# tarepan/DDSP-SVC-official

Measured on AMD Instinct MI355X. Metric: audio samples/sec @44.1kHz CombSub synth, higher is better.
Workload: dtype f32 storage and accumulation; products of the GEMM / FIR contractions split-bf16x3 (hi*hi+hi*lo+lo*hi), of the attention split-bf16 from three pieces (6 products) for the feature projections and two (3 products) for the context sums; everything else f32; `value_fp32_mfma` is the leg with every produ; 1 GPU; CombSub 44.1 kHz, batch=64x2 s per GPU (Fr=172, T=88064), units/f0/volume/spk_id -> audio, seeded random weights, in-kernel noise

## Files before the change

ddsp-svc-official_amd/csrc/fir_synth.hip:

```cpp
#include "gemm_f32.h"
#include "tables.h"

#include <stdlib.h>

namespace {

__global__ void __launch_bounds__(256) fir_act_kernel(int mode, const float* __restrict__ ctrl, int64_t ld, int M,
                                                      int ldo, int64_t rows, float* __restrict__ out, int split) {
    const int lane = threadIdx.x & 63;
    const int64_t row = (int64_t)blockIdx.x * 4 + (threadIdx.x >> 6);
    if (row >= rows) return;
    const float* src = ctrl + row * ld;
    if (mode != DDSP_FIR_ALLPASS) {
        float* dst = out + row * ldo;
        const float scale = (mode == DDSP_FIR_STATIC) ? (1.0f / 128.0f) : 1.0f;
        if (split) {
            for (int f0 = 0; f0 < M; f0 += 64) {
                const int f = f0 + lane;
                const float v = f < M ? expf(src[f]) * scale : 0.f;
                const uint32_t w = ddsp_split1_group8(v, lane);
                if (f < M) ((uint32_t*)dst)[f] = w;
            }
            return;
        }
        for (int f = lane; f < M; f += 64) dst[f] = expf(src[f]) * scale;
        return;
    }
    float* dst = out + row * ldo;
    const float pi_f = 3.14159274101257324f;
    double carry = 0.0;
    for (int f0 = 0; f0 < M; f0 += 64) {
        const int f = f0 + lane;
        const float gd = (f < M) ? __fmul_rn(pi_f, tanhf(src[f])) : 0.f;
        double incl = (double)gd;
#pragma unroll
        for (int o = 1; o < 64; o <<= 1) {
            double nb = __shfl_up(incl, o, 64);
            if (lane >= o) incl += nb;
        }
        const float phi = (float)(carry + incl);
        carry += __shfl(incl, 63, 64);
        float s = 0.f, c = 0.f;
        if (f < M) sincosf(phi, &s, &c);
        if (split) {
            const uint32_t wc = ddsp_split1_group8(c, lane), ws = ddsp_split1_group8(s, lane);
            if (f < M) {
                ((uint32_t*)dst)[f] = wc;
                ((uint32_t*)dst)[M + f] = ws;
            }
        } else if (f < M) {
            dst[f] = c;
            dst[M + f] = s;
        }
    }
}

struct EpiDynWindow {
    float* ir;
    int n;
    const float* f0;
    float sr15;
    int fast;
    __device__ __forceinline__ float col(int) const { return 0.f; }
    __device__ __forceinline__ float window_fast(float inv_hw, int k) const {
        float w = (float)(k - n / 2) * inv_hw;
        if (w > 1.0f) w = 0.0f;
        return fmaf(0.5f, __builtin_amdgcn_cosf(0.5f * w), 0.5f);
    }
    __device__ __forceinline__ float window(float hw, int k) const {
        float w = __fdiv_rn((float)(k - n / 2), hw);
        if (w > 1.0f) w = 0.0f;
        return __fdiv_rn(__fadd_rn(1.0f, cosf(__fmul_rn(3.14159274101257324f, w))), 2.0f);
    }
    __device__ __forceinline__ void operator()(int, int m, int k, float v, float) const {
        float* row = ir + (int64_t)m * n;
        if (fast) {
            const float inv_hw = __fdiv_rn(__fadd_rn(f0[m], 1e-3f), sr15);
            row[k] = v * window_fast(inv_hw, k);
            if (k > 0 && k < n / 2) row[n - k] = v * window_fast(inv_hw, n - k);
            return;
        }
        const float hw = __fdiv_rn(sr15, __fadd_rn(f0[m], 1e-3f));
        row[k] = __fmul_rn(v, window(hw, k));
        if (k > 0 && k < n / 2) row[n - k] = __fmul_rn(v, window(hw, n - k));
    }
};

struct EpiMirrorStore {
    float* ir;
    int n;
    __device__ __forceinline__ float col(int) const { return 0.f; }
    __device__ __forceinline__ void operator()(int, int m, int k, float v, float) const {
        float* row = ir + (int64_t)m * n;
        row[k] = v;
        if (k > 0 && k < n / 2) row[n - k] = v;
    }
};


__global__ void __launch_bounds__(256) fir_act_exp8_kernel(float scale, const float* __restrict__ ctrl, int64_t ld, int M, int ldo,
                                                           int64_t rows, float* __restrict__ out, int split) {
    const int per_row = M / 8;
    const int64_t i = (int64_t)blockIdx.x * 256 + threadIdx.x;
    if (i >= rows * per_row) return;
    const int64_t row = i / per_row;
    const int gq = (int)(i % per_row);
    const float* src = ctrl + row * ld + 8 * gq;
    const f32x4 a = *(const f32x4*)src, b = *(const f32x4*)(src + 4);
    float v[8];
#pragma unroll
    for (int e = 0; e < 4; ++e) {
        v[e] = expf(a[e]) * scale;
        v[4 + e] = expf(b[e]) * scale;
    }
    float* dst = out + row * ldo + 8 * gq;
    if (split) {
        ddsp_u32x4 hi, lo;
        ddsp_split8(v, hi, lo);
        *(ddsp_u32x4*)dst = hi;
        *(ddsp_u32x4*)(dst + 4) = lo;
    } else {
        *(f32x4*)dst = f32x4{v[0], v[1], v[2], v[3]};
        *(f32x4*)(dst + 4) = f32x4{v[4], v[5], v[6], v[7]};
    }
}

template <int CTRL, int ROW_MASK>
__device__ __forceinline__ double act_dpp_d(double v) {
    const uint64_t u = __builtin_bit_cast(uint64_t, v);
    const int lo = __builtin_amdgcn_update_dpp(0, (int)(uint32_t)u, CTRL, ROW_MASK, 0xf, false);
    const int hi = __builtin_amdgcn_update_dpp(0, (int)(uint32_t)(u >> 32), CTRL, ROW_MASK, 0xf, false);
    return __builtin_bit_cast(double, ((uint64_t)(uint32_t)hi << 32) | (uint32_t)lo);
}
__global__ void __launch_bounds__(256) fir_act_allpass4_kernel(const float* __restrict__ ctrl, int64_t ld, int M, int ldo, int64_t rows,
                                                               float* __restrict__ out, int split) {
    const int lane = threadIdx.x & 63;
    const int64_t row = (int64_t)blockIdx.x * 4 + (threadIdx.x >> 6);
    if (row >= rows) return;
    const float* src = ctrl + row * ld;
    float* dst = out + row * ldo;
    const float pi_f = 3.14159274101257324f;
    double carry = 0.0;
    for (int f0 = 0; f0 < M; f0 += 256) {
        const int f = f0 + 4 * lane;
        const bool in = f < M;
        f32x4 x = {0.f, 0.f, 0.f, 0.f};
        if (in) x = *(const f32x4*)(src + f);
        double run = 0.0, loc[4];
#pragma unroll
        for (int e = 0; e < 4; ++e) {
            const float gd = in ? __fmul_rn(pi_f, tanhf(x[e])) : 0.f;
            run += (double)gd;
            loc[e] = run;
        }
        double incl = run;
        incl += act_dpp_d<0x111, 0xf>(incl);
        incl += act_dpp_d<0x112, 0xf>(incl);
        incl += act_dpp_d<0x114, 0xf>(incl);
        incl += act_dpp_d<0x118, 0xf>(incl);
        incl += act_dpp_d<0x142, 0xa>(incl);
        incl += act_dpp_d<0x143, 0xc>(incl);
        const double base = carry + (incl - run);
        f32x4 c, sn;
#pragma unroll
        for (int e = 0; e < 4; ++e) {
            const float phi = (float)(base + loc[e]);
            float s_ = 0.f, c_ = 0.f;
            if (in) sincosf(phi, &s_, &c_);
            c[e] = c_;
            sn[e] = s_;
        }
        {
            const uint64_t u = __builtin_bit_cast(uint64_t, incl);
            const uint32_t lo = __builtin_amdgcn_readlane((int)(uint32_t)u, 63), hi = __builtin_amdgcn_readlane((int)(uint32_t)(u >> 32), 63);
            carry += __builtin_bit_cast(double, ((uint64_t)hi << 32) | lo);
        }
        if (split) {
            const ddsp_u32x4 pc = ddsp_split4_pair(c, (lane & 1) != 0, 1), ps = ddsp_split4_pair(sn, (lane & 1) != 0, 1);
            if (in) {
                *(ddsp_u32x4*)(dst + f) = pc;
                *(ddsp_u32x4*)(dst + M + f) = ps;
            }
        } else if (in) {
            *(f32x4*)(dst + f) = c;
            *(f32x4*)(dst + M + f) = sn;
        }
    }
}

__global__ void __launch_bounds__(256) repack_rows_kernel(const float* __restrict__ src, int n, int64_t rows, int ld,
                                                          float* __restrict__ dst) {
    typedef float f32x2r __attribute__((ext_vector_type(2)));
    const int half = ld / 2;
    const int64_t total = rows * half;
    for (int64_t i = (int64_t)blockIdx.x * blockDim.x + threadIdx.x; i < total; i += (int64_t)gridDim.x * blockDim.x) {
        const int64_t m = i / half;
        const int k = 2 * (int)(i % half);
        f32x2r v = {0.f, 0.f};
        if (k < n) v = *(const f32x2r*)(src + m * n + k);
        *(f32x2r*)(dst + m * ld + k) = v;
    }
}

__global__ void __launch_bounds__(256) dyn_window_scale_kernel(float* __restrict__ d_ir, const float* __restrict__ f0,
                                                               int n, int64_t rows, float sr15) {
    const int64_t total = rows * n;
    for (int64_t i = (int64_t)blockIdx.x * blockDim.x + threadIdx.x; i < total; i += (int64_t)gridDim.x * blockDim.x) {
        const int64_t m = i / n;
        const int k = (int)(i % n);
        const float hw = __fdiv_rn(sr15, __fadd_rn(f0[m], 1e-3f));
        float w = __fdiv_rn((float)(k - n / 2), hw);
        if (w > 1.0f) w = 0.0f;
        d_ir[i] *= __fdiv_rn(__fadd_rn(1.0f, cosf(__fmul_rn(3.14159274101257324f, w))), 2.0f);
    }
}

__global__ void __launch_bounds__(256) fir_act_bwd_kernel(int mode, const float* __restrict__ ctrl, int64_t ld, int M,
                                                          const float* __restrict__ d_act, int lda, int64_t rows,
// ... 38 lines not shown
    }
    float tail = 0.f;
#pragma unroll
    for (int c = 15; c >= 0; --c) {
        if (c < nchunk) {
            float incl = dphi[c];
#pragma unroll
            for (int o = 1; o < 64; o <<= 1) {
                float nb = __shfl_down(incl, o, 64);
                if (lane + o < 64) incl += nb;
            }
            const float G = incl + tail;
            tail += __shfl(incl, 0, 64);
            const int f = c * 64 + lane;
            if (f < M) dst[f] = G * pi_f * (1.0f - th[c] * th[c]);
        }
    }
}

}


extern "C" int ddsp_fir_from_ctrl(ddsp_ctx* ctx, void* stream, int mode, const float* ctrl, int64_t ctrl_ld,
                                  int n_mag, const float* f0_frames, int64_t rows, int sr, float* ir) {
    DDSP_REQUIRE(ctx, ctx && ctrl && ir, "ddsp_fir_from_ctrl: null argument");
    DDSP_REQUIRE(ctx, mode >= 0 && mode <= 2, "ddsp_fir_from_ctrl: unknown mode");
    DDSP_REQUIRE(ctx, n_mag >= 3 && n_mag <= 1024 && ctrl_ld >= n_mag && rows >= 0 && rows < (1 << 30),
                 "ddsp_fir_from_ctrl: bad shape");
    DDSP_REQUIRE(ctx, mode != DDSP_FIR_DYNAMIC || f0_frames, "ddsp_fir_from_ctrl: DYNAMIC needs f0_frames");
    if (rows == 0) return DDSP_OK;
    hipStream_t st = (hipStream_t)stream;
    DDSP_ENTER_DEVICE(ctx);
    const int M = n_mag, n = 2 * (n_mag - 1);
    const int K = (mode == DDSP_FIR_ALLPASS) ? 2 * M : M;
    const int lda = ddsp_pad4(K);
    int rc = ddsp_scratch_reserve_bytes(ctx, (size_t)rows * lda * sizeof(float) + 4096);
    if (rc) return rc;
    ddsp_scratch_reset(ctx);
    float* act = nullptr;
    rc = ddsp_scratch_get(ctx, (size_t)rows * lda * sizeof(float), (void**)&act);
    if (rc) return rc;
    float* tab = nullptr;
    const int kind = mode == DDSP_FIR_ALLPASS ? TAB_IRDFT_CPLX : (mode == DDSP_FIR_STATIC ? TAB_IRDFT_RE_HANN : TAB_IRDFT_RE);
    const bool tap_major = K % 32 == 0;
    rc = ddsp_get_table(ctx, st, kind, M, tap_major ? 1 : 0, &tab);
    if (rc) return rc;
    float* tab_split = nullptr;
    if (tap_major && ctx->math != DDSP_MATH_FP32 && (rc = ddsp_get_table(ctx, st, kind, M, 2, &tab_split))) return rc;

    const bool presplit = tap_major && tab_split && rows >= 8192 && M % 8 == 0 && ctx->math != 4;
    ddsp_prof_begin(ctx, st, PF_FIR_ACT);
    const bool wide = M % 8 == 0 && ctrl_ld % 4 == 0 && lda % 8 == 0 && ((uintptr_t)ctrl % 16) == 0;
    if (wide && mode != DDSP_FIR_ALLPASS)
        hipLaunchKernelGGL(fir_act_exp8_kernel, dim3((unsigned)ceil_div64(rows * (M / 8), 256)), dim3(256), 0, st,
                           mode == DDSP_FIR_STATIC ? 1.0f / 128.0f : 1.0f, ctrl, ctrl_ld, M, lda, rows, act, presplit ? 1 : 0);
    else if (wide)
        hipLaunchKernelGGL(fir_act_allpass4_kernel, dim3((unsigned)ceil_div64(rows, 4)), dim3(256), 0, st, ctrl, ctrl_ld, M, lda, rows,
                           act, presplit ? 1 : 0);
    else
        hipLaunchKernelGGL(fir_act_kernel, dim3((unsigned)ceil_div64(rows, 4)), dim3(256), 0, st, mode, ctrl, ctrl_ld, M,
                           lda, rows, act, presplit ? 1 : 0);
    ddsp_prof_end(ctx, st, 0.0, 4.0 * rows * (M + K));
    DDSP_LAUNCH_CHECK(ctx);
    ddsp_prof_begin(ctx, st, PF_FIR_DFT_GEMM);

    auto run = [&](gemm::Args g, const auto& epi) {
        g.math = tap_major ? (ctx->math == 4 ? DDSP_MATH_SPLIT_BF16 : ctx->math) : 0;
        g.B_split = tab_split;
        if (presplit) {
            g.A_split = 1;
            g.B = tab_split;
        }
        if (tap_major)
            gemm::launch<true, true, gemm::A_PLAIN>(st, g, 1, epi);
        else
            gemm::launch<true, false, gemm::A_PLAIN>(st, g, 1, epi);
    };
    const int64_t ldb = tap_major ? K : ddsp_pad4(n);
    if (mode == DDSP_FIR_ALLPASS) {
        gemm::Args g = gemm::make(act, lda, tab, ldb, (int)rows, n, K);
        run(g, gemm::EpiStore{ir, n, nullptr, 1, 0, 0});
    } else {
        gemm::Args g = gemm::make(act, lda, tab, ldb, (int)rows, n / 2 + 1, K);
        if (mode == DDSP_FIR_DYNAMIC)
            run(g, EpiDynWindow{ir, n, f0_frames, 1.5f * (float)sr, (tap_major && ctx->math != DDSP_MATH_FP32) ? 1 : 0});
        else
            run(g, EpiMirrorStore{ir, n});
    }
    ddsp_prof_end(ctx, st, 2.0 * rows * (double)n * K, 4.0 * rows * (K + n));
    DDSP_LAUNCH_CHECK(ctx);
    return DDSP_OK;
}

extern "C" int ddsp_fir_from_ctrl_bwd(ddsp_ctx* ctx, void* stream, int mode, const float* ctrl, int64_t ctrl_ld,
                                      int n_mag, const float* f0_frames, int64_t rows, int sr, float* d_ir,
                                      float* d_ctrl, int64_t d_ctrl_ld) {
    DDSP_REQUIRE(ctx, ctx && ctrl && d_ir && d_ctrl, "ddsp_fir_from_ctrl_bwd: null argument");
    DDSP_REQUIRE(ctx, mode >= 0 && mode <= 2, "ddsp_fir_from_ctrl_bwd: unknown mode");
    DDSP_REQUIRE(ctx, n_mag >= 3 && n_mag <= 1024 && ctrl_ld >= n_mag && d_ctrl_ld >= n_mag && rows >= 0 && rows < (1 << 30),
                 "ddsp_fir_from_ctrl_bwd: bad shape");
    DDSP_REQUIRE(ctx, mode != DDSP_FIR_DYNAMIC || f0_frames, "ddsp_fir_from_ctrl_bwd: DYNAMIC needs f0_frames");
    if (rows == 0) return DDSP_OK;
    hipStream_t st = (hipStream_t)stream;
    DDSP_ENTER_DEVICE(ctx);
    const int M = n_mag, n = 2 * (n_mag - 1);
    const int K = (mode == DDSP_FIR_ALLPASS) ? 2 * M : M;
    const int lda = ddsp_pad4(K);
    const int ldp = ddsp_pad4(n);
    const bool repack = ctx->math != DDSP_MATH_FP32 && ldp % 32 == 0 && rows >= 1024;
    int rc = ddsp_scratch_reserve_bytes(ctx, (size_t)rows * (lda + (repack ? ldp : 0)) * sizeof(float) + 8192);
    if (rc) return rc;
    ddsp_scratch_reset(ctx);
    float* d_act = nullptr;
    if ((rc = ddsp_scratch_get(ctx, (size_t)rows * lda * sizeof(float), (void**)&d_act))) return rc;
    float* d_pad = nullptr;
    if (repack && (rc = ddsp_scratch_get(ctx, (size_t)rows * ldp * sizeof(float), (void**)&d_pad))) return rc;
    float* tab = nullptr;
    const int kind = mode == DDSP_FIR_ALLPASS ? TAB_IRDFT_CPLX : (mode == DDSP_FIR_STATIC ? TAB_IRDFT_RE_HANN : TAB_IRDFT_RE);
    if ((rc = ddsp_get_table(ctx, st, kind, M, 0, &tab))) return rc;
    ddsp_prof_begin(ctx, st, PF_FIR_SYNTH_BWD);
    if (mode == DDSP_FIR_DYNAMIC) {
        int64_t blocks = ceil_div64(rows * n, 256);
// ... 23 lines not shown
```

ddsp-svc-official_amd/csrc/gemm_f32.h:

```cpp
#pragma once
#include "common.h"

#include <stdlib.h>
#include <type_traits>

namespace gemm {

enum { A_PLAIN = 0, A_CONV3 = 1, A_FRAMES = 2, A_CONVK = 3 };

struct Args {
    const float* A;
    const float* B;
    int M, N, K;
    int64_t lda, ldb;
    int zdiv;
    int64_t sA_hi, sA_lo, sB_hi, sB_lo;
    int Fr, Cin;
    int tap_shift;
    int ktaps, dil;
    float in_slope;
    const float* zeros;
    int sub_from, parent_tn;
    int math;
    const float* B_split;
    int A_split;
    int xcd;
    int xcd_cut;
    int kz;
};

constexpr int BK = 32;
typedef float f32x4_u __attribute__((ext_vector_type(4), aligned(4)));

template <class E, class = void>
struct epi_wants_pair : std::false_type {};
template <class E>
struct epi_wants_pair<E, std::void_t<decltype(E::kPair)>> : std::true_type {};
template <class E, class = void>
struct epi_has_store4 : std::false_type {};
template <class E>
struct epi_has_store4<E, std::void_t<decltype(E::kStore4)>> : std::true_type {};

template <class E, class = void>
struct epi_is_gated : std::false_type {};
template <class E>
struct epi_is_gated<E, std::void_t<decltype(E::kGatedPair)>> : std::true_type {};

template <class E, class = void>
struct epi_is_rowpair : std::false_type {};
template <class E>
struct epi_is_rowpair<E, std::void_t<decltype(E::kRowPair)>> : std::true_type {};

__device__ __forceinline__ void quad_transpose(float (&x)[4], int q) {
    const bool odd = q & 1, hi = q & 2;
    auto swap1 = [](float v) { return __builtin_bit_cast(float, __builtin_amdgcn_mov_dpp(__builtin_bit_cast(int, v), 0xB1, 0xF, 0xF, true)); };
    auto swap2 = [](float v) { return __builtin_bit_cast(float, __builtin_amdgcn_mov_dpp(__builtin_bit_cast(int, v), 0x4E, 0xF, 0xF, true)); };
    const float r0 = swap1(odd ? x[0] : x[1]);
    const float r1 = swap1(odd ? x[2] : x[3]);
    const float a_lo = odd ? r0 : x[0], a_hi = odd ? x[1] : r0;
    const float b_lo = odd ? r1 : x[2], b_hi = odd ? x[3] : r1;
    const float s_lo = swap2(hi ? a_lo : b_lo);
    const float s_hi = swap2(hi ? a_hi : b_hi);
    x[0] = hi ? s_lo : a_lo;
    x[1] = hi ? s_hi : a_hi;
    x[2] = hi ? b_lo : s_lo;
    x[3] = hi ? b_hi : s_hi;
}

template <int BM, int BN, bool A_KC, bool B_KC, int A_MODE, class Epi, int NW = 4>
__global__ void __launch_bounds__(64 * NW) kernel(Args g, Epi epi) {
    constexpr int WGM = NW / 2, WGN = 2, NT = 64 * NW;
    constexpr int TM = BM / (32 * WGM), TN = BN / (32 * WGN);
    static_assert(TM >= 1 && TN >= 1, "tile too small for the wave grid");
    constexpr int LDM = BM + 1, LDN = BN + 1;
    __shared__ float lds[2 * BK * (LDM + LDN)];
    float* const As0 = lds;
    float* const Bs0 = lds + 2 * BK * LDM;

    const int tid = threadIdx.x;
    const int lane = tid & 63;
    const int wave = tid >> 6;
    const int wm = (wave >> 1) * (BM / WGM);
    const int wn = (wave & 1) * (BN / WGN);
    const int m0 = blockIdx.y * BM;
    const int n0 = blockIdx.x * BN;
// ... 116 lines not shown
            if (A_KC) {
                const int r = q / (BK / 4), kq = q % (BK / 4);
#pragma unroll
                for (int j = 0; j < 4; ++j) as[(kq * 4 + j) * LDM + r] = ra[i][j];
            } else {
                const int kr = q / (BM / 4), mq = q % (BM / 4);
#pragma unroll
                for (int j = 0; j < 4; ++j) as[kr * LDM + mq * 4 + j] = ra[i][j];
            }
        }
#pragma unroll
        for (int i = 0; i < NB; ++i) {
            const int q = tid + i * NT;
            if (B_KC) {
                const int r = q / (BK / 4), kq = q % (BK / 4);
#pragma unroll
                for (int j = 0; j < 4; ++j) bs[(kq * 4 + j) * LDN + r] = rb[i][j];
            } else {
                const int kr = q / (BN / 4), nq = q % (BN / 4);
#pragma unroll
                for (int j = 0; j < 4; ++j) bs[kr * LDN + nq * 4 + j] = rb[i][j];
            }
        }
    };

    f32x16 acc[TM][TN];
#pragma unroll
    for (int i = 0; i < TM; ++i)
#pragma unroll
        for (int j = 0; j < TN; ++j)
#pragma unroll
            for (int r = 0; r < 16; ++r) acc[i][j][r] = 0.f;

    const int nk = (g.K + BK - 1) / BK;
    load_tiles(0);
    store_tiles(0);
    __syncthreads();
    const int lr = lane & 31, lh = lane >> 5;
    for (int kt = 0; kt < nk; ++kt) {
        const int buf = kt & 1;
        if (kt + 1 < nk) load_tiles((kt + 1) * BK);
        const float* as = As0 + buf * (BK * LDM) + wm + lr + lh * LDM;
        const float* bs = Bs0 + buf * (BK * LDN) + wn + lr + lh * LDN;
        float a[TM], b[TN];
#pragma unroll
        for (int i = 0; i < TM; ++i) a[i] = as[32 * i];
#pragma unroll
        for (int j = 0; j < TN; ++j) b[j] = bs[32 * j];
#pragma unroll
        for (int kk = 0; kk < BK; kk += 2) {
            float an[TM], bn[TN];
            if (kk + 2 < BK) {
#pragma unroll
                for (int i = 0; i < TM; ++i) an[i] = as[(kk + 2) * LDM + 32 * i];
#pragma unroll
                for (int j = 0; j < TN; ++j) bn[j] = bs[(kk + 2) * LDN + 32 * j];
            }
#pragma unroll
            for (int i = 0; i < TM; ++i)
#pragma unroll
                for (int j = 0; j < TN; ++j)
                    acc[i][j] = __builtin_amdgcn_mfma_f32_32x32x2f32(a[i], b[j], acc[i][j], 0, 0, 0);
            if (kk + 2 < BK) {
#pragma unroll
                for (int i = 0; i < TM; ++i) a[i] = an[i];
#pragma unroll
                for (int j = 0; j < TN; ++j) b[j] = bn[j];
            }
        }
        if (kt + 1 < nk) store_tiles(buf ^ 1);
        __syncthreads();
    }

#pragma unroll
    for (int i = 0; i < TM; ++i)
#pragma unroll
        for (int j = 0; j < TN; ++j) {
            const int n = n0 + wn + 32 * j + lr;
            const bool n_ok = n < g.N;
            const float cb = n_ok ? epi.col(n) : 0.f;
#pragma unroll
            for (int r = 0; r < 16; ++r) {
                const int m = m0 + wm + 32 * i + (r & 3) + 8 * (r >> 2) + 4 * lh;
                if constexpr (epi_is_rowpair<Epi>::value) {
                    if ((r & 1) == 0 && n_ok && m < g.M) epi.pair(z, m, n, acc[i][j][r], acc[i][j][r + 1], cb);
                } else if constexpr (epi_wants_pair<Epi>::value) {
                    const float other = __shfl_xor(acc[i][j][r], 1, 64);
                    if (n_ok && m < g.M) epi(z, m, n, acc[i][j][r], other);
                } else {
                    if (n_ok && m < g.M) epi(z, m, n, acc[i][j][r], cb);
                }
            }
        }
}


template <int BM, int BN, class Epi, int NS = 3, int NW = 8, int A_MODE = A_PLAIN, int MATH = 0>
__global__ void __launch_bounds__(64 * NW, (NW == 4 ? 3 : BM * BN <= 128 * 128 ? 4 : 2)) kernel_dma(Args g, Epi epi, int tiles_m, int tiles_n, int total_tiles) {
    constexpr int WGM = NW / 2, WGN = 2;
    constexpr int TM = BM / (32 * WGM), TN = BN / (32 * WGN);
    constexpr int ROWS = BM + BN;
    constexpr int STAGE = ROWS * 32;
    constexpr int PIECES = ROWS / 8;
    constexpr int PPW = PIECES / NW;
    static_assert(PIECES % NW == 0, "stage must split evenly over the waves");
    __shared__ __attribute__((aligned(1024))) float lds[NS * STAGE];

    const int tid = threadIdx.x, lane = tid & 63, wave = __builtin_amdgcn_readfirstlane(tid >> 6);
    const int wm = (wave >> 1) * (BM / WGM), wn = (wave & 1) * (BN / WGN);
    const int lr = lane & 31, lh = lane >> 5;
    const int nk = g.K / 32;

    const bool xcd_order = g.xcd && (gridDim.x & 7) == 0 && g.sub_from == 0 && total_tiles == tiles_m * tiles_n - g.xcd_cut;
    const int xq0 = (int)blockIdx.x >> 3, xgs = (int)gridDim.x >> 3, xx = (int)blockIdx.x & 7;
    const int xown = (tiles_m / 8) * tiles_n, xleft = (tiles_m % 8) * tiles_n - g.xcd_cut;
    int my_tiles = (total_tiles - (int)blockIdx.x + (int)gridDim.x - 1) / (int)gridDim.x;
    if (xcd_order) {
// ... 79 lines not shown
                }
            }
            __builtin_amdgcn_global_load_lds((const __attribute__((address_space(1))) void*)p,
                                             (__attribute__((address_space(3))) void*)(lds + stage * STAGE + piece * 256),
                                             16, 0, 0);
        }
    };

    const float* src_cur[PPW];
    int issued = 0;
    int issue_tile = 0, issue_kt = 0;
    if (steps > 0) tile_src(tile_of(0), src_cur);
    auto issue_next = [&]() {
        if (issued >= steps) return;
        issue(src_cur, issue_kt, issued % NS);
        ++issued;
        if (++issue_kt == nk) {
            issue_kt = 0;
            ++issue_tile;
            if (issue_tile < my_tiles) tile_src(tile_of(issue_tile), src_cur);
        }
    };
#pragma unroll
    for (int i = 0; i < NS - 1; ++i) issue_next();

    f32x16 acc[TM][TN];
#pragma unroll
    for (int i = 0; i < TM; ++i)
#pragma unroll
        for (int j = 0; j < TN; ++j)
#pragma unroll
            for (int r = 0; r < 16; ++r) acc[i][j][r] = 0.f;

    int kt = 0, tile_i = 0;
    for (int step = 0; step < steps; ++step) {
        static_assert((NS - 2) * PPW <= 63, "vmcnt is a 6-bit counter");
        if (NS > 2 && step + NS - 2 < steps)
            asm volatile("s_waitcnt vmcnt(%0)" ::"n"((NS - 2) * PPW) : "memory");
        else
            asm volatile("s_waitcnt vmcnt(0)" ::: "memory");
        __builtin_amdgcn_s_barrier();
        issue_next();
        const float* st = lds + (step % NS) * STAGE;
        f32x4 av[TM][4], bv[TN][4];
#pragma unroll
        for (int i = 0; i < TM; ++i) {
            const int row = wm + 32 * i + lr;
            const float* rp = st + row * 32;
#pragma unroll
            for (int c = 0; c < 4; ++c) av[i][c] = *(const f32x4*)(rp + 4 * ((4 * lh + c) ^ ((row >> 1) & 7)));
        }
#pragma unroll
        for (int j = 0; j < TN; ++j) {
            const int row = BM + wn + 32 * j + lr;
            const float* rp = st + row * 32;
#pragma unroll
            for (int c = 0; c < 4; ++c) bv[j][c] = *(const f32x4*)(rp + 4 * ((4 * lh + c) ^ ((row >> 1) & 7)));
        }
        if constexpr (MATH != 0) {
            typedef __bf16 bf16x8 __attribute__((ext_vector_type(8)));
            typedef float f32x2p __attribute__((ext_vector_type(2)));
            typedef __bf16 bf16x2p __attribute__((ext_vector_type(2)));
            typedef uint32_t u32x4p __attribute__((ext_vector_type(4)));
            auto split = [](const f32x4& x0, const f32x4& x1, bf16x8 (&p)[3]) {
                constexpr int NQ = 2;
                u32x4p w[3];
// ... 23 lines not shown
                        split(av[i][2 * half], av[i][2 * half + 1], ap[i]);
                    }
                }
#pragma unroll
                for (int j = 0; j < TN; ++j) {
                    if constexpr (MATH == 7 || MATH == 8) {
                        bp[j][0] = __builtin_bit_cast(bf16x8, bv[j][2 * half]);
                        bp[j][1] = __builtin_bit_cast(bf16x8, bv[j][2 * half + 1]);
                    } else {
                        split(bv[j][2 * half], bv[j][2 * half + 1], bp[j]);
                    }
                }
#pragma unroll
                for (int i = 0; i < TM; ++i)
#pragma unroll
                    for (int j = 0; j < TN; ++j) {
                        auto mm = [&](int x, int y) {
                            acc[i][j] = __builtin_amdgcn_mfma_f32_32x32x16_bf16(ap[i][x], bp[j][y], acc[i][j], 0, 0, 0);
                        };
                        mm(1, 0);
                        mm(0, 1);
                        mm(0, 0);
                    }
            }
        } else {
#pragma unroll
            for (int s = 0; s < 16; ++s)
#pragma unroll
                for (int i = 0; i < TM; ++i)
#pragma unroll
                    for (int j = 0; j < TN; ++j)
                        acc[i][j] = __builtin_amdgcn_mfma_f32_32x32x2f32(av[i][s >> 2][s & 3], bv[j][s >> 2][s & 3],
                                                                         acc[i][j], 0, 0, 0);
        }
        if (++kt == nk) {
            const int tile = tile_of(tile_i);
            const int per_z = tiles_m * tiles_n;
            int z = tile / per_z, rem = tile - z * per_z;
            int m0 = (rem / tiles_n) * BM, n0 = (rem % tiles_n) * BN;
            if (g.sub_from > 0) {
                const int big = g.sub_from + (tile >> 2), q = tile & 3;
                z = 0;
                m0 = (2 * (big / g.parent_tn) + (q >> 1)) * BM;
                n0 = (2 * (big % g.parent_tn) + (q & 1)) * BN;
            }
            bool vec = false;
            if constexpr (epi_has_store4<Epi>::value) vec = epi.vec_ok() && n0 + BN <= g.N;
            if constexpr (epi_is_gated<Epi>::value) {
                static_assert(TN == 2, "gated-pair epilogue needs the wave's two column blocks");
                const int q = lane & 3;
                const int na = n0 + wn + lr;
                const float ba = epi.col(na), bg = epi.col(na + 32);
                const int oc = ((n0 + wn) >> 1) + (lr & ~3);
#pragma unroll
                for (int i = 0; i < TM; ++i)
#pragma unroll
                    for (int rg = 0; rg < 4; ++rg) {
                        float x[4];
#pragma unroll
                        for (int r = 0; r < 4; ++r) {
                            const float a = acc[i][0][4 * rg + r] + ba, gt = acc[i][1][4 * rg + r] + bg;
                            if constexpr (MATH != 0)
                                x[r] = a * __builtin_amdgcn_rcpf(1.0f + __builtin_amdgcn_exp2f(-1.44269504088896341f * gt));
                            else
                                x[r] = a * (1.0f / (1.0f + expf(-gt)));
                            acc[i][0][4 * rg + r] = 0.f;
// ... 3 lines not shown
                        const int m = m0 + wm + 32 * i + q + 8 * rg + 4 * lh;
                        if (m < g.M) epi.store4(z, m, oc, f32x4{x[0], x[1], x[2], x[3]});
                    }
            } else if (vec) {
                if constexpr (epi_has_store4<Epi>::value) {
                    const int q = lane & 3;
#pragma unroll
                    for (int i = 0; i < TM; ++i)
#pragma unroll
                        for (int j = 0; j < TN; ++j) {
                            const int n = n0 + wn + 32 * j + (lr & ~3);
#pragma unroll
                            for (int rg = 0; rg < 4; ++rg) {
                                float x[4] = {acc[i][j][4 * rg], acc[i][j][4 * rg + 1], acc[i][j][4 * rg + 2], acc[i][j][4 * rg + 3]};
                                quad_transpose(x, q);
                                const int m = m0 + wm + 32 * i + q + 8 * rg + 4 * lh;
                                if (m < g.M) epi.store4(z, m, n, f32x4{x[0], x[1], x[2], x[3]});
#pragma unroll
                                for (int r = 0; r < 4; ++r) acc[i][j][4 * rg + r] = 0.f;
                            }
                        }
                }
            } else
#pragma unroll
            for (int i = 0; i < TM; ++i)
#pragma unroll
                for (int j = 0; j < TN; ++j) {
                    const int n = n0 + wn + 32 * j + lr;
                    const bool n_ok = n < g.N;
                    const float cb = n_ok ? epi.col(n) : 0.f;
#pragma unroll
                    for (int r = 0; r < 16; ++r) {
                        const int m = m0 + wm + 32 * i + (r & 3) + 8 * (r >> 2) + 4 * lh;
                        if constexpr (epi_is_rowpair<Epi>::value) {
                            if ((r & 1) == 0 && n_ok && m < g.M) epi.pair(z, m, n, acc[i][j][r], acc[i][j][r + 1], cb);
                        } else if constexpr (epi_wants_pair<Epi>::value) {
                            const float other = __shfl_xor(acc[i][j][r], 1, 64);
                            if (n_ok && m < g.M) epi(z, m, n, acc[i][j][r], other);
                        } else {
                            if (n_ok && m < g.M) epi(z, m, n, acc[i][j][r], cb);
                        }
                        acc[i][j][r] = 0.f;
                    }
                }
            kt = 0;
            ++tile_i;
        }
    }
}

inline bool dma_ok(const Args& g) {
    return g.K % 32 == 0 && g.lda % 4 == 0 && g.ldb % 4 == 0 && ((uintptr_t)g.A % 16) == 0 && ((uintptr_t)g.B % 16) == 0 &&
           g.sA_hi % 4 == 0 && g.sA_lo % 4 == 0 && g.sB_hi % 4 == 0 && g.sB_lo % 4 == 0;
}

template <int BM, int BN, class Epi, int NS = 3, int NW = 8, int A_MODE = A_PLAIN, int MATH = 0>
inline void launch_dma(hipStream_t st, const Args& g, int batch, const Epi& epi, int total_override = -1) {
    const int tiles_m = (g.M + BM - 1) / BM, tiles_n = (g.N + BN - 1) / BN;
    const int total = total_override >= 0 ? total_override : tiles_m * tiles_n * batch;
    if (total == 0) return;
    constexpr int lds_bytes = NS * (BM + BN) * 128;
    constexpr int by_waves = 16 / NW;
    constexpr int by_lds = 160 * 1024 / lds_bytes;
    constexpr int per_cu = by_lds < by_waves ? by_lds : by_waves;
    int grid = 256 * per_cu;
    if (grid > total) grid = total;
    hipLaunchKernelGGL((kernel_dma<BM, BN, Epi, NS, NW, A_MODE, MATH>), dim3(grid), dim3(64 * NW), 0, st, g, epi, tiles_m, tiles_n, total);
// ... 171 lines not shown
```

ddsp-svc-official_amd/csrc/tables.h:

```cpp
#pragma once
#include "common.h"

enum {
    TAB_IRDFT_RE = 1,
    TAB_IRDFT_RE_HANN = 2,
    TAB_IRDFT_CPLX = 3,
    TAB_RDFT_FWD_W = 4,
    TAB_RDFT_INV_W = 5,
    TAB_F0_AC = 6,
};

static inline int ddsp_pad4(int n) { return (n + 3) & ~3; }
```

ddsp-svc-official_amd/csrc/tables.hip:

```cpp
#include "tables.h"

namespace {

constexpr double kTwoPi = 6.283185307179586476925286766559;

__global__ void irdft_table_kernel(float* __restrict__ tab, int M, int n, int ld, int rows, int hann, int tap_major) {
    const int64_t total = tap_major ? (int64_t)n * rows : (int64_t)rows * ld;
    for (int64_t idx = (int64_t)blockIdx.x * blockDim.x + threadIdx.x; idx < total;
         idx += (int64_t)gridDim.x * blockDim.x) {
        const int row = tap_major ? (int)(idx % rows) : (int)(idx / ld);
        const int k = tap_major ? (int)(idx / rows) : (int)(idx % ld);
        if (k >= n) {
            tab[idx] = 0.f;
            continue;
        }
        const int f = row < M ? row : row - M;
        const double cf = (f == 0 || f == M - 1) ? 1.0 : 2.0;
        int64_t r = ((int64_t)f * (k - n / 2)) % n;
        if (r < 0) r += n;
        const double ang = kTwoPi * (double)r / (double)n;
        double v;
        if (row < M)
            v = cf / n * cos(ang);
        else
            v = (f == 0 || f == M - 1) ? 0.0 : -cf / n * sin(ang);
        if (hann) v *= 0.5 - 0.5 * cos(kTwoPi * (double)k / (double)n);
        tab[idx] = (float)v;
    }
}

__global__ void rdft_w_table_kernel(float* __restrict__ tab, int N, int ld, int inverse) {
    const int Mb = N / 2 + 1;
    const int64_t total = inverse ? (int64_t)N * 2 * Mb : (int64_t)N * ld;
    for (int64_t idx = (int64_t)blockIdx.x * blockDim.x + threadIdx.x; idx < total;
         idx += (int64_t)gridDim.x * blockDim.x) {
        int i, col;
        if (!inverse) {
            i = (int)(idx / ld);
            col = (int)(idx % ld);
            if (col >= 2 * Mb) {
                tab[idx] = 0.f;
                continue;
            }
        } else {
            col = (int)(idx / N);
            i = (int)(idx % N);
        }
        const int f = col < Mb ? col : col - Mb;
        const bool im = col >= Mb;
        const int64_t r = ((int64_t)f * i) % N;
        const double ang = kTwoPi * (double)r / (double)N;
        const double w = sqrt(0.5 - 0.5 * cos(kTwoPi * (double)i / (double)N));
        double v;
        if (!inverse) {
            v = im ? -sin(ang) : cos(ang);
// ... 40 lines not shown
    if (ctx->n_tables >= 64) return ddsp_fail(ctx, DDSP_ERR_OOM, "table cache full", "");
    if (n1 == 2) {
        float* plain = nullptr;
        int rc = ddsp_get_table(ctx, st, kind, n0, 1, &plain);
        if (rc) return rc;
        if (ctx->n_tables >= 64) return ddsp_fail(ctx, DDSP_ERR_OOM, "table cache full", "");
        size_t bytes = 0;
        for (int i = 0; i < ctx->n_tables; ++i)
            if (ctx->tables[i].dev == plain) bytes = ctx->tables[i].bytes;
        if (bytes == 0 || bytes % 32 != 0) return ddsp_fail(ctx, DDSP_ERR_ARG, "table cannot be pre-split", "");
        float* dev = nullptr;
        hipError_t e = hipMalloc((void**)&dev, bytes);
        if (e != hipSuccess) return ddsp_fail(ctx, DDSP_ERR_OOM, "table hipMalloc", hipGetErrorString(e));
        const int64_t groups = (int64_t)(bytes / 32);
        hipLaunchKernelGGL(presplit_kernel, dim3((unsigned)((groups + 255) / 256 > 2048 ? 2048 : (groups + 255) / 256)), dim3(256), 0,
                           st, plain, (uint32_t*)dev, groups);
        DDSP_LAUNCH_CHECK(ctx);
        ddsp_table& t = ctx->tables[ctx->n_tables++];
        t.kind = kind;
        t.n0 = n0;
        t.n1 = n1;
        t.dev = dev;
        t.bytes = bytes;
        *out = dev;
        return DDSP_OK;
    }
    size_t elems = 0;
    switch (kind) {
        case TAB_IRDFT_RE:
        case TAB_IRDFT_RE_HANN:
            elems = n1 ? (size_t)n0 * 2 * (n0 - 1) : (size_t)n0 * ddsp_pad4(2 * (n0 - 1));
            break;
        case TAB_IRDFT_CPLX:
            elems = n1 ? (size_t)2 * n0 * 2 * (n0 - 1) : (size_t)2 * n0 * ddsp_pad4(2 * (n0 - 1));
            break;
        case TAB_RDFT_FWD_W:
            elems = (size_t)n0 * ddsp_pad4(2 * (n0 / 2 + 1));
            break;
        case TAB_RDFT_INV_W:
            elems = (size_t)n0 * 2 * (n0 / 2 + 1);
            break;
        default:
            return ddsp_fail(ctx, DDSP_ERR_ARG, "unknown table kind", "");
    }
    float* dev = nullptr;
    hipError_t e = hipMalloc((void**)&dev, elems * sizeof(float));
    if (e != hipSuccess) return ddsp_fail(ctx, DDSP_ERR_OOM, "table hipMalloc", hipGetErrorString(e));
    const unsigned blocks = (unsigned)((elems + 255) / 256 > 2048 ? 2048 : (elems + 255) / 256);
    if (kind == TAB_IRDFT_RE || kind == TAB_IRDFT_RE_HANN || kind == TAB_IRDFT_CPLX) {
        const int M = n0, n = 2 * (n0 - 1);
        const int rows = kind == TAB_IRDFT_CPLX ? 2 * M : M;
        hipLaunchKernelGGL(irdft_table_kernel, dim3(blocks), dim3(256), 0, st, dev, M, n, ddsp_pad4(n), rows,
                           kind == TAB_IRDFT_RE_HANN ? 1 : 0, n1 ? 1 : 0);
    } else {
        hipLaunchKernelGGL(rdft_w_table_kernel, dim3(blocks), dim3(256), 0, st, dev, n0,
                           ddsp_pad4(2 * (n0 / 2 + 1)), kind == TAB_RDFT_INV_W ? 1 : 0);
    }
    DDSP_LAUNCH_CHECK(ctx);
    ddsp_table& t = ctx->tables[ctx->n_tables++];
    t.kind = kind;
    t.n0 = n0;
    t.n1 = n1;
    t.dev = dev;
    t.bytes = elems * sizeof(float);
    *out = dev;
    return DDSP_OK;
}
```

Baseline: 4.936 billion samples/s.

## Exploit even/odd symmetry in allpass IRDFT GEMM to halve output columns

For the allpass FIR mode, the complex IRDFT GEMM now computes only n/2+1 output taps. It accumulates the cosine half and the sine half of K into separate accumulators, then writes e+o and e-o to the mirrored tap positions in a dual epilogue. The frequency dimension is padded to a multiple of 32 so the K split lands on a tile boundary, and the table generator is changed to match the new layout. This roughly halves the GEMM FLOPs for the allpass path, at the cost of extra accumulator registers (acc1) that may reduce occupancy, plus padding work.

```diff
diff --git a/ddsp-svc-official_amd/csrc/fir_synth.hip b/ddsp-svc-official_amd/csrc/fir_synth.hip
--- a/ddsp-svc-official_amd/csrc/fir_synth.hip
+++ b/ddsp-svc-official_amd/csrc/fir_synth.hip
@@ -5,7 +5,7 @@
 
 namespace {
 
-__global__ void __launch_bounds__(256) fir_act_kernel(int mode, const float* __restrict__ ctrl, int64_t ld, int M,
+__global__ void __launch_bounds__(256) fir_act_kernel(int mode, const float* __restrict__ ctrl, int64_t ld, int M, int Mp,
                                                       int ldo, int64_t rows, float* __restrict__ out, int split) {
     const int lane = threadIdx.x & 63;
     const int64_t row = (int64_t)blockIdx.x * 4 + (threadIdx.x >> 6);
@@ -29,7 +29,7 @@
     float* dst = out + row * ldo;
     const float pi_f = 3.14159274101257324f;
     double carry = 0.0;
-    for (int f0 = 0; f0 < M; f0 += 64) {
+    for (int f0 = 0; f0 < Mp; f0 += 64) {
         const int f = f0 + lane;
         const float gd = (f < M) ? __fmul_rn(pi_f, tanhf(src[f])) : 0.f;
         double incl = (double)gd;
@@ -44,13 +44,13 @@
         if (f < M) sincosf(phi, &s, &c);
         if (split) {
             const uint32_t wc = ddsp_split1_group8(c, lane), ws = ddsp_split1_group8(s, lane);
-            if (f < M) {
+            if (f < Mp) {
                 ((uint32_t*)dst)[f] = wc;
-                ((uint32_t*)dst)[M + f] = ws;
-            }
-        } else if (f < M) {
+                ((uint32_t*)dst)[Mp + f] = ws;
+            }
+        } else if (f < Mp) {
             dst[f] = c;
-            dst[M + f] = s;
+            dst[Mp + f] = s;
         }
     }
 }
@@ -97,6 +97,17 @@
     }
 };
 
+struct EpiEvenOdd {
+    float* ir;
+    int n;
+    static constexpr bool kDual = true;
+    __device__ __forceinline__ float col(int) const { return 0.f; }
+    __device__ __forceinline__ void operator()(int, int m, int k, float e, float o) const {
+        float* row = ir + (int64_t)m * n;
+        row[k] = e + o;
+        if (k > 0 && k < n / 2) row[n - k] = e - o;
+    }
+};
 
 __global__ void __launch_bounds__(256) fir_act_exp8_kernel(float scale, const float* __restrict__ ctrl, int64_t ld, int M, int ldo,
                                                            int64_t rows, float* __restrict__ out, int split) {
@@ -132,8 +143,8 @@
     const int hi = __builtin_amdgcn_update_dpp(0, (int)(uint32_t)(u >> 32), CTRL, ROW_MASK, 0xf, false);
     return __builtin_bit_cast(double, ((uint64_t)(uint32_t)hi << 32) | (uint32_t)lo);
 }
-__global__ void __launch_bounds__(256) fir_act_allpass4_kernel(const float* __restrict__ ctrl, int64_t ld, int M, int ldo, int64_t rows,
-                                                               float* __restrict__ out, int split) {
+__global__ void __launch_bounds__(256) fir_act_allpass4_kernel(const float* __restrict__ ctrl, int64_t ld, int M, int Mp, int ldo,
+                                                               int64_t rows, float* __restrict__ out, int split) {
     const int lane = threadIdx.x & 63;
     const int64_t row = (int64_t)blockIdx.x * 4 + (threadIdx.x >> 6);
     if (row >= rows) return;
@@ -141,9 +152,9 @@
     float* dst = out + row * ldo;
     const float pi_f = 3.14159274101257324f;
     double carry = 0.0;
-    for (int f0 = 0; f0 < M; f0 += 256) {
+    for (int f0 = 0; f0 < Mp; f0 += 256) {
         const int f = f0 + 4 * lane;
-        const bool in = f < M;
+        const bool in = f < M, st = f < Mp;
         f32x4 x = {0.f, 0.f, 0.f, 0.f};
         if (in) x = *(const f32x4*)(src + f);
         double run = 0.0, loc[4];
@@ -177,13 +188,13 @@
         }
         if (split) {
             const ddsp_u32x4 pc = ddsp_split4_pair(c, (lane & 1) != 0, 1), ps = ddsp_split4_pair(sn, (lane & 1) != 0, 1);
-            if (in) {
+            if (st) {
                 *(ddsp_u32x4*)(dst + f) = pc;
-                *(ddsp_u32x4*)(dst + M + f) = ps;
-            }
-        } else if (in) {
+                *(ddsp_u32x4*)(dst + Mp + f) = ps;
+            }
+        } else if (st) {
             *(f32x4*)(dst + f) = c;
-            *(f32x4*)(dst + M + f) = sn;
+            *(f32x4*)(dst + Mp + f) = sn;
         }
     }
 }
@@ -288,7 +299,8 @@
     hipStream_t st = (hipStream_t)stream;
     DDSP_ENTER_DEVICE(ctx);
     const int M = n_mag, n = 2 * (n_mag - 1);
-    const int K = (mode == DDSP_FIR_ALLPASS) ? 2 * M : M;
+    const int Mp = ddsp_pad32(M);
+    const int K = (mode == DDSP_FIR_ALLPASS) ? 2 * Mp : M;
     const int lda = ddsp_pad4(K);
     int rc = ddsp_scratch_reserve_bytes(ctx, (size_t)rows * lda * sizeof(float) + 4096);
     if (rc) return rc;
@@ -301,27 +313,29 @@
     const bool tap_major = K % 32 == 0;
     rc = ddsp_get_table(ctx, st, kind, M, tap_major ? 1 : 0, &tab);
     if (rc) return rc;
+    const bool bf16_ok = tap_major && (mode != DDSP_FIR_ALLPASS || M % 16 == 0);
     float* tab_split = nullptr;
-    if (tap_major && ctx->math != DDSP_MATH_FP32 && (rc = ddsp_get_table(ctx, st, kind, M, 2, &tab_split))) return rc;
-
-    const bool presplit = tap_major && tab_split && rows >= 8192 && M % 8 == 0 && ctx->math != 4;
+    if (bf16_ok && ctx->math != DDSP_MATH_FP32 && (rc = ddsp_get_table(ctx, st, kind, M, 2, &tab_split))) return rc;
+
+    const bool presplit = tap_major && tab_split && rows >= 8192 && M % 8 == 0 && ctx->math != 4 &&
+                          (mode != DDSP_FIR_ALLPASS || K >= 256);
     ddsp_prof_begin(ctx, st, PF_FIR_ACT);
     const bool wide = M % 8 == 0 && ctrl_ld % 4 == 0 && lda % 8 == 0 && ((uintptr_t)ctrl % 16) == 0;
     if (wide && mode != DDSP_FIR_ALLPASS)
         hipLaunchKernelGGL(fir_act_exp8_kernel, dim3((unsigned)ceil_div64(rows * (M / 8), 256)), dim3(256), 0, st,
                            mode == DDSP_FIR_STATIC ? 1.0f / 128.0f : 1.0f, ctrl, ctrl_ld, M, lda, rows, act, presplit ? 1 : 0);
     else if (wide)
-        hipLaunchKernelGGL(fir_act_allpass4_kernel, dim3((unsigned)ceil_div64(rows, 4)), dim3(256), 0, st, ctrl, ctrl_ld, M, lda, rows,
-                           act, presplit ? 1 : 0);
+        hipLaunchKernelGGL(fir_act_allpass4_kernel, dim3((unsigned)ceil_div64(rows, 4)), dim3(256), 0, st, ctrl, ctrl_ld, M, Mp, lda,
+                           rows, act, presplit ? 1 : 0);
     else
-        hipLaunchKernelGGL(fir_act_kernel, dim3((unsigned)ceil_div64(rows, 4)), dim3(256), 0, st, mode, ctrl, ctrl_ld, M,
+        hipLaunchKernelGGL(fir_act_kernel, dim3((unsigned)ceil_div64(rows, 4)), dim3(256), 0, st, mode, ctrl, ctrl_ld, M, Mp,
                            lda, rows, act, presplit ? 1 : 0);
     ddsp_prof_end(ctx, st, 0.0, 4.0 * rows * (M + K));
     DDSP_LAUNCH_CHECK(ctx);
     ddsp_prof_begin(ctx, st, PF_FIR_DFT_GEMM);
 
     auto run = [&](gemm::Args g, const auto& epi) {
-        g.math = tap_major ? (ctx->math == 4 ? DDSP_MATH_SPLIT_BF16 : ctx->math) : 0;
+        g.math = bf16_ok ? (ctx->math == 4 ? DDSP_MATH_SPLIT_BF16 : ctx->math) : 0;
         g.B_split = tab_split;
         if (presplit) {
             g.A_split = 1;
@@ -334,8 +348,8 @@
     };
     const int64_t ldb = tap_major ? K : ddsp_pad4(n);
     if (mode == DDSP_FIR_ALLPASS) {
-        gemm::Args g = gemm::make(act, lda, tab, ldb, (int)rows, n, K);
-        run(g, gemm::EpiStore{ir, n, nullptr, 1, 0, 0});
+        gemm::Args g = gemm::make(act, lda, tab, ldb, (int)rows, n / 2 + 1, K);
+        run(g, EpiEvenOdd{ir, n});
     } else {
         gemm::Args g = gemm::make(act, lda, tab, ldb, (int)rows, n / 2 + 1, K);
         if (mode == DDSP_FIR_DYNAMIC)
@@ -343,7 +357,8 @@
         else
             run(g, EpiMirrorStore{ir, n});
     }
-    ddsp_prof_end(ctx, st, 2.0 * rows * (double)n * K, 4.0 * rows * (K + n));
+    ddsp_prof_end(ctx, st, mode == DDSP_FIR_ALLPASS ? 2.0 * rows * (double)(n / 2 + 1) * 2 * M : 2.0 * rows * (double)n * K,
+                  4.0 * rows * (K + n));
     DDSP_LAUNCH_CHECK(ctx);
     return DDSP_OK;
 }
diff --git a/ddsp-svc-official_amd/csrc/gemm_f32.h b/ddsp-svc-official_amd/csrc/gemm_f32.h
--- a/ddsp-svc-official_amd/csrc/gemm_f32.h
+++ b/ddsp-svc-official_amd/csrc/gemm_f32.h
@@ -51,6 +51,11 @@
 template <class E>
 struct epi_is_rowpair<E, std::void_t<decltype(E::kRowPair)>> : std::true_type {};
 
+template <class E, class = void>
+struct epi_is_dual : std::false_type {};
+template <class E>
+struct epi_is_dual<E, std::void_t<decltype(E::kDual)>> : std::true_type {};
+
 __device__ __forceinline__ void quad_transpose(float (&x)[4], int q) {
     const bool odd = q & 1, hi = q & 2;
     auto swap1 = [](float v) { return __builtin_bit_cast(float, __builtin_amdgcn_mov_dpp(__builtin_bit_cast(int, v), 0xB1, 0xF, 0xF, true)); };
@@ -233,6 +238,8 @@
 #pragma unroll
             for (int r = 0; r < 16; ++r) acc[i][j][r] = 0.f;
 
+    constexpr bool DUAL = epi_is_dual<Epi>::value;
+    f32x16 acc1[DUAL ? TM : 1][DUAL ? TN : 1];
     const int nk = (g.K + BK - 1) / BK;
     load_tiles(0);
     store_tiles(0);
@@ -269,6 +276,18 @@
                 for (int j = 0; j < TN; ++j) b[j] = bn[j];
             }
         }
+        if constexpr (DUAL) {
+            if (2 * (kt + 1) == nk) {
+#pragma unroll
+                for (int i = 0; i < TM; ++i)
+#pragma unroll
+                    for (int j = 0; j < TN; ++j) {
+                        acc1[i][j] = acc[i][j];
+#pragma unroll
+                        for (int r = 0; r < 16; ++r) acc[i][j][r] = 0.f;
+                    }
+            }
+        }
         if (kt + 1 < nk) store_tiles(buf ^ 1);
         __syncthreads();
     }
@@ -283,7 +302,9 @@
 #pragma unroll
             for (int r = 0; r < 16; ++r) {
                 const int m = m0 + wm + 32 * i + (r & 3) + 8 * (r >> 2) + 4 * lh;
-                if constexpr (epi_is_rowpair<Epi>::value) {
+                if constexpr (DUAL) {
+                    if (n_ok && m < g.M) epi(z, m, n, acc1[i][j][r], acc[i][j][r]);
+                } else if constexpr (epi_is_rowpair<Epi>::value) {
                     if ((r & 1) == 0 && n_ok && m < g.M) epi.pair(z, m, n, acc[i][j][r], acc[i][j][r + 1], cb);
                 } else if constexpr (epi_wants_pair<Epi>::value) {
                     const float other = __shfl_xor(acc[i][j][r], 1, 64);
@@ -429,6 +450,9 @@
 #pragma unroll
             for (int r = 0; r < 16; ++r) acc[i][j][r] = 0.f;
 
+    constexpr bool DUAL = epi_is_dual<Epi>::value;
+    f32x16 acc1[DUAL ? TM : 1][DUAL ? TN : 1];
+
     int kt = 0, tile_i = 0;
     for (int step = 0; step < steps; ++step) {
         static_assert((NS - 2) * PPW <= 63, "vmcnt is a 6-bit counter");
@@ -518,6 +542,18 @@
                     for (int j = 0; j < TN; ++j)
                         acc[i][j] = __builtin_amdgcn_mfma_f32_32x32x2f32(av[i][s >> 2][s & 3], bv[j][s >> 2][s & 3],
                                                                          acc[i][j], 0, 0, 0);
+        }
+        if constexpr (DUAL) {
+            if (2 * (kt + 1) == nk) {
+#pragma unroll
+                for (int i = 0; i < TM; ++i)
+#pragma unroll
+                    for (int j = 0; j < TN; ++j) {
+                        acc1[i][j] = acc[i][j];
+#pragma unroll
+                        for (int r = 0; r < 16; ++r) acc[i][j][r] = 0.f;
+                    }
+            }
         }
         if (++kt == nk) {
             const int tile = tile_of(tile_i);
@@ -587,7 +623,9 @@
 #pragma unroll
                     for (int r = 0; r < 16; ++r) {
                         const int m = m0 + wm + 32 * i + (r & 3) + 8 * (r >> 2) + 4 * lh;
-                        if constexpr (epi_is_rowpair<Epi>::value) {
+                        if constexpr (DUAL) {
+                            if (n_ok && m < g.M) epi(z, m, n, acc1[i][j][r], acc[i][j][r]);
+                        } else if constexpr (epi_is_rowpair<Epi>::value) {
                             if ((r & 1) == 0 && n_ok && m < g.M) epi.pair(z, m, n, acc[i][j][r], acc[i][j][r + 1], cb);
                         } else if constexpr (epi_wants_pair<Epi>::value) {
                             const float other = __shfl_xor(acc[i][j][r], 1, 64);
diff --git a/ddsp-svc-official_amd/csrc/tables.h b/ddsp-svc-official_amd/csrc/tables.h
--- a/ddsp-svc-official_amd/csrc/tables.h
+++ b/ddsp-svc-official_amd/csrc/tables.h
@@ -11,3 +11,4 @@
 };
 
 static inline int ddsp_pad4(int n) { return (n + 3) & ~3; }
+static inline int ddsp_pad32(int n) { return (n + 31) & ~31; }
diff --git a/ddsp-svc-official_amd/csrc/tables.hip b/ddsp-svc-official_amd/csrc/tables.hip
--- a/ddsp-svc-official_amd/csrc/tables.hip
+++ b/ddsp-svc-official_amd/csrc/tables.hip
@@ -4,23 +4,24 @@
 
 constexpr double kTwoPi = 6.283185307179586476925286766559;
 
-__global__ void irdft_table_kernel(float* __restrict__ tab, int M, int n, int ld, int rows, int hann, int tap_major) {
-    const int64_t total = tap_major ? (int64_t)n * rows : (int64_t)rows * ld;
+__global__ void irdft_table_kernel(float* __restrict__ tab, int M, int n, int ld, int rows, int half, int taps, int hann,
+                                   int tap_major) {
+    const int64_t total = tap_major ? (int64_t)taps * rows : (int64_t)rows * ld;
     for (int64_t idx = (int64_t)blockIdx.x * blockDim.x + threadIdx.x; idx < total;
          idx += (int64_t)gridDim.x * blockDim.x) {
         const int row = tap_major ? (int)(idx % rows) : (int)(idx / ld);
         const int k = tap_major ? (int)(idx / rows) : (int)(idx % ld);
-        if (k >= n) {
+        const int f = row < half ? row : row - half;
+        if (k >= n || f >= M) {
             tab[idx] = 0.f;
             continue;
         }
-        const int f = row < M ? row : row - M;
         const double cf = (f == 0 || f == M - 1) ? 1.0 : 2.0;
         int64_t r = ((int64_t)f * (k - n / 2)) % n;
         if (r < 0) r += n;
         const double ang = kTwoPi * (double)r / (double)n;
         double v;
-        if (row < M)
+        if (row < half)
             v = cf / n * cos(ang);
         else
             v = (f == 0 || f == M - 1) ? 0.0 : -cf / n * sin(ang);
@@ -127,7 +128,7 @@
             elems = n1 ? (size_t)n0 * 2 * (n0 - 1) : (size_t)n0 * ddsp_pad4(2 * (n0 - 1));
             break;
         case TAB_IRDFT_CPLX:
-            elems = n1 ? (size_t)2 * n0 * 2 * (n0 - 1) : (size_t)2 * n0 * ddsp_pad4(2 * (n0 - 1));
+            elems = n1 ? (size_t)n0 * 2 * ddsp_pad32(n0) : (size_t)2 * n0 * ddsp_pad4(2 * (n0 - 1));
             break;
         case TAB_RDFT_FWD_W:
             elems = (size_t)n0 * ddsp_pad4(2 * (n0 / 2 + 1));
@@ -144,9 +145,10 @@
     const unsigned blocks = (unsigned)((elems + 255) / 256 > 2048 ? 2048 : (elems + 255) / 256);
     if (kind == TAB_IRDFT_RE || kind == TAB_IRDFT_RE_HANN || kind == TAB_IRDFT_CPLX) {
         const int M = n0, n = 2 * (n0 - 1);
-        const int rows = kind == TAB_IRDFT_CPLX ? 2 * M : M;
-        hipLaunchKernelGGL(irdft_table_kernel, dim3(blocks), dim3(256), 0, st, dev, M, n, ddsp_pad4(n), rows,
-                           kind == TAB_IRDFT_RE_HANN ? 1 : 0, n1 ? 1 : 0);
+        const bool cplx = kind == TAB_IRDFT_CPLX;
+        const int half = cplx && n1 ? ddsp_pad32(M) : M;
+        hipLaunchKernelGGL(irdft_table_kernel, dim3(blocks), dim3(256), 0, st, dev, M, n, ddsp_pad4(n), cplx ? 2 * half : M, half,
+                           cplx ? n / 2 + 1 : n, kind == TAB_IRDFT_RE_HANN ? 1 : 0, n1 ? 1 : 0);
     } else {
         hipLaunchKernelGGL(rdft_w_table_kernel, dim3(blocks), dim3(256), 0, st, dev, n0,
                            ddsp_pad4(2 * (n0 / 2 + 1)), kind == TAB_RDFT_INV_W ? 1 : 0);
```

Result: faster. 5.021 billion samples/s (median of 6 runs) (+1.7%).
